# htcr/sam_road

Measured on AMD Instinct MI355X. Metric: tiles/sec (512x512 ViT-B, SAMRoad.infer_masks_and_img_features: encoder + mask decoder), higher is better.
Workload: dtype f16; 1 GPU; toponet_vitb_512_cityscale.yaml, batch=16 512x512 tiles per GPU, ViT-B encoder + map_decoder (BASELINE configs[1]); patch=512, input=f32 NHWC resident in HBM, weights=seeded random init, parallelism=tile-dp1

## Files before the change

include/samroad_hip.h:

```cpp
#ifndef SAMROAD_HIP_H
#define SAMROAD_HIP_H

#include <stddef.h>
#include <stdint.h>

#ifdef __cplusplus
extern "C" {
#endif

#define SRH_ABI_VERSION 11

typedef enum {
    SRH_OK = 0,
    SRH_ERR_BAD_ARG = -1,
    SRH_ERR_UNSUPPORTED = -2,
    SRH_ERR_HIP = -3,
    SRH_ERR_MISSING_WEIGHT = -4,
    SRH_ERR_NO_DEVICE = -5,
    SRH_ERR_NONFINITE = -6
} srh_status;

typedef enum { SRH_F32 = 0, SRH_F16 = 1, SRH_U8 = 2, SRH_I32 = 3, SRH_I64 = 4 } srh_dtype;

typedef struct srh_ctx srh_ctx;
// ... 68 lines not shown
                           int fill_b, void* stream);
int srh_scene_normalise_valid_hw(srh_ctx* ctx, const float* canvas_kp, const float* canvas_road, int H, int W,
                                 const int32_t* tile_xy, int n_tiles, int P, const uint8_t* valid, uint8_t* kp_u8,
                                 uint8_t* road_u8, void* stream);

int srh_scene_pass1_window_hw(srh_ctx* ctx, const srh_weights* w, const uint8_t* scene, int H, int W, const int32_t* tile_xy,
                              int n_tiles, int B, const float* profile, float* canvas_kp, float* canvas_road,
                              float* embeddings_all, void* stream);
int srh_scene_normalise_window_hw(srh_ctx* ctx, const float* canvas_kp, const float* canvas_road, int H, int W,
                                  const int32_t* tile_xy, int n_tiles, int P, const float* profile, const uint8_t* valid,
                                  uint8_t* kp_u8, uint8_t* road_u8, void* stream);
int srh_op_scene_fuse_window(srh_ctx* ctx, const float* scores, int n, int P, const int32_t* tile_xy, const float* profile,
                             float* canvas_kp, float* canvas_road, int H, int W, void* stream);

int srh_scene_pass1_tta_hw(srh_ctx* ctx, const srh_weights* w, const uint8_t* scene, int H, int W, const int32_t* tile_xy,
                           int n_tiles, int B, const uint8_t* orients, int k, const float* profile, float* canvas_kp,
                           float* canvas_road, float* embeddings_all, void* stream);
int srh_op_patch_im2col(srh_ctx* ctx, const uint8_t* scene_u8, int H, int W, const int32_t* tile_xy, int n, int P, int orient,
                        void* out_f16, void* stream);
int srh_op_scores_unorient(srh_ctx* ctx, const float* scores_in, int n, int P, int orient, float* scores_out, void* stream);


int srh_op_gemm(srh_ctx* ctx, const void* A_f16, const void* W_f16, const float* bias, const float* resid,
                int M, int N, int K, int act, float* out_f32, void* out_f16, void* stream);
#define SRH_GEMM_A_BLOCKED16 1
#define SRH_GEMM_OUT_BLOCKED16 2
int srh_op_gemm_ex(srh_ctx* ctx, const void* A_f16, const void* W_f16, const float* bias, const float* resid,
                   int M, int N, int K, int act, float* out_f32, void* out_f16, int flags, void* stream);
size_t srh_ctx_device_bytes(const srh_ctx* ctx);
int srh_op_conv3x3(srh_ctx* ctx, const void* A_f16, const void* W_f16, int B, int S, int C, int N,
                   float* out_f32, void* stream);
int srh_op_layernorm(srh_ctx* ctx, const float* x, const float* gamma, const float* beta, float eps, int M,
                     int D, int gelu, float* out_f32, void* out_f16, void* stream);
int srh_op_attention(srh_ctx* ctx, const void* qkv_f16, const void* relpos_h_f16, const void* relpos_w_f16,
                     const void* bias_qkv_f16, int B, int S, int heads, int win, void* out_f16, void* stream);
int srh_op_attention_hd(srh_ctx* ctx, const void* qkv_f16, const void* relpos_h_f16, const void* relpos_w_f16,
                        const void* bias_qkv_f16, int B, int S, int heads, int head_dim, int win,
                        void* out_f16, void* stream);

int srh_op_map_decoder(srh_ctx* ctx, const srh_weights* w, const void* emb_f16, int B, float* mask_logits, float* mask_scores, void* stream);
int srh_op_sample(srh_ctx* ctx, const float* emb_f32, int n_tiles, int h, int w, int C, const void* points, int points_dtype,
                  const int32_t* point_tile, int B, int N, float patch, float* out_f32, void* out_f16, void* stream);
int srh_op_pair_gather(srh_ctx* ctx, const void* pf_f16, const void* points, int points_dtype, const void* pairs, int pairs_dtype,
                       int B, int N, int Ns, int K, int zero_offset, int64_t index_base, void* out_f16, int ld, void* stream);


typedef struct {
    char name[32];
    int64_t launches;
    double ms;
    double flops;
    double bytes;
} srh_profile_row;
int srh_profile_enable(srh_ctx* ctx, int on);
int srh_profile_read(srh_ctx* ctx, srh_profile_row* rows, int max_rows, int* n_rows);
int srh_profile_overhead(srh_ctx* ctx, void* stream, double* ms_per_launch);

int srh_nms_points_host(const int32_t* xy, const uint8_t* force, int64_t n, int32_t radius, uint8_t* kept);

int srh_pass2_count(const int64_t* pts, int64_t n, const int32_t* boxes, int32_t n_tiles, int64_t* counts);
int srh_pass2_fill(const int64_t* pts, int64_t n, const int32_t* boxes, int32_t n_tiles, int32_t K, int64_t radius,
                   const int64_t* offsets, int64_t* ids, int32_t* knn, uint8_t* ambiguous, int64_t* local, int32_t n_threads);

int srh_kdtree_knn_host(const double* points, int64_t n, int32_t leafsize, const double* queries, int64_t nq, int32_t k,
                        double distance_upper_bound, int32_t* out_idx, int32_t* tree_indices);

// ... 32 lines not shown
```

sam_road_amd/_lib.py:

```python
import ctypes as C
import os

_HERE = os.path.dirname(os.path.abspath(__file__))
LIB_PATH = os.environ.get("SRH_LIB_PATH") or os.path.join(_HERE, "libsamroad_hip.so")

SRH_F32, SRH_F16, SRH_U8, SRH_I32, SRH_I64 = 0, 1, 2, 3, 4
ABI_VERSION = 11
SRH_GEMM_A_BLOCKED16, SRH_GEMM_OUT_BLOCKED16 = 1, 2


class SrhError(RuntimeError):
    pass


class ModelCfg(C.Structure):
    _fields_ = [("embed_dim", C.c_int32), ("depth", C.c_int32), ("num_heads", C.c_int32),
                ("patch_size", C.c_int32), ("n_global", C.c_int32), ("global_attn_indexes", C.c_int32 * 8),
                ("window_size", C.c_int32), ("toponet_version", C.c_int32), ("use_sam_decoder", C.c_int32)]


class NamedTensor(C.Structure):
    _fields_ = [("name", C.c_char_p), ("data", C.c_void_p), ("on_device", C.c_int32), ("ndim", C.c_int32),
                ("shape", C.c_int64 * 4)]

# ... 4 lines not shown


_P, _I, _F = C.c_void_p, C.c_int, C.c_float
SYMBOLS = {
    "srh_abi_version": (_I, []),
    "srh_build_id": (C.c_char_p, []),
    "srh_ctx_create": (_I, [_I, C.POINTER(_P)]),
    "srh_ctx_destroy": (None, [_P]),
    "srh_last_error": (C.c_char_p, [_P]),
    "srh_weights_pack": (_I, [_P, C.POINTER(ModelCfg), C.POINTER(NamedTensor), _I, C.POINTER(_P)]),
    "srh_weights_free": (None, [_P]),
    "srh_weights_export": (_I, [_P, _P, _P, C.c_size_t, C.POINTER(C.c_size_t)]),
    "srh_weights_import": (_I, [_P, C.POINTER(ModelCfg), _P, C.c_size_t, C.POINTER(_P)]),
    "srh_encode_decode": (_I, [_P, _P, _P, _I, _I, _P, _P, _P, _P]),
    "srh_toponet": (_I, [_P, _P, _P, _P, _I, _P, _I, _P, _I, _I, _I, _I, _P, _P, _P]),
    "srh_scene_pass1": (_I, [_P, _P, _P, _I, _P, _I, _I, _P, _P, _P, _P]),
    "srh_scene_normalise": (_I, [_P, _P, _P, _I, _P, _I, _I, _P, _P, _P]),
    "srh_scene_pass1_hw": (_I, [_P, _P, _P, _I, _I, _P, _I, _I, _P, _P, _P, _P]),
    "srh_scene_normalise_hw": (_I, [_P, _P, _P, _I, _I, _P, _I, _I, _P, _P, _P]),
    "srh_scene_tile_valid": (_I, [_P, _P, _I, _I, _P, _I, _I, _P, _P]),
    "srh_scene_fill_invalid": (_I, [_P, _P, _P, _I, _I, _I, _I, _I, _P]),
    "srh_scene_normalise_valid_hw": (_I, [_P, _P, _P, _I, _I, _P, _I, _I, _P, _P, _P, _P]),
    "srh_scene_pass1_window_hw": (_I, [_P, _P, _P, _I, _I, _P, _I, _I, _P, _P, _P, _P, _P]),
    "srh_scene_normalise_window_hw": (_I, [_P, _P, _P, _I, _I, _P, _I, _I, _P, _P, _P, _P, _P]),
    "srh_op_scene_fuse_window": (_I, [_P, _P, _I, _I, _P, _P, _P, _P, _I, _I, _P]),
    "srh_scene_pass1_tta_hw": (_I, [_P, _P, _P, _I, _I, _P, _I, _I, _P, _I, _P, _P, _P, _P, _P]),
    "srh_op_patch_im2col": (_I, [_P, _P, _I, _I, _P, _I, _I, _I, _P, _P]),
    "srh_op_scores_unorient": (_I, [_P, _P, _I, _I, _I, _P, _P]),
    "srh_op_gemm": (_I, [_P, _P, _P, _P, _P, _I, _I, _I, _I, _P, _P, _P]),
    "srh_op_gemm_ex": (_I, [_P, _P, _P, _P, _P, _I, _I, _I, _I, _P, _P, _I, _P]),
    "srh_ctx_device_bytes": (C.c_size_t, [_P]),
    "srh_op_conv3x3": (_I, [_P, _P, _P, _I, _I, _I, _I, _P, _P]),
    "srh_op_layernorm": (_I, [_P, _P, _P, _P, _F, _I, _I, _I, _P, _P, _P]),
    "srh_op_attention": (_I, [_P, _P, _P, _P, _P, _I, _I, _I, _I, _P, _P]),
    "srh_op_attention_hd": (_I, [_P, _P, _P, _P, _P, _I, _I, _I, _I, _I, _P, _P]),
    "srh_op_map_decoder": (_I, [_P, _P, _P, _I, _P, _P, _P]),
    "srh_op_sample": (_I, [_P, _P, _I, _I, _I, _I, _P, _I, _P, _I, _I, _F, _P, _P, _P]),
    "srh_op_pair_gather": (_I, [_P, _P, _P, _I, _P, _I, _I, _I, _I, _I, _I, C.c_int64, _P, _I, _P]),
    "srh_nms_points_host": (_I, [_P, _P, C.c_int64, C.c_int32, _P]),
    "srh_pass2_count": (_I, [_P, C.c_int64, _P, C.c_int32, _P]),
    "srh_pass2_fill": (_I, [_P, C.c_int64, _P, C.c_int32, C.c_int32, C.c_int64, _P, _P, _P, _P, _P, C.c_int32]),
    "srh_pass2_votes": (_I, [_P, C.c_int32, C.c_int64, C.c_int32, _P, _P, _P, C.c_int64, _P, _P, C.c_int64, _P]),
    "srh_pass2_vote_sums": (_I, [_P, _P, _P, _P, C.c_int32, C.c_int32, _P, C.c_int32, _P, _P, C.c_int64, _P, _P, _P, _P, C.c_int64, _P, C.c_int32]),
    "srh_votes_to_edges": (_I, [_P, _P, _P, _P, C.c_int64, C.c_int64, C.c_double, _P, _P]),
    "srh_pass2_pack": (_I, [_P, _P, _P, C.c_int32, C.c_int64, C.c_int32, _P, _P, _P]),
    "srh_pass2_pack_ragged": (_I, [_P, _P, _P, C.c_int32, C.c_int32, _P, _P, _P, _P]),
    "srh_toponet_ragged": (_I, [_P, _P, _P, _I, _P, _P, _P, _P, C.c_int64, _I, _P, _P, _P]),
    "srh_ctx_check": (_I, [_P, _P, _I]),
    "srh_kdtree_knn_host": (_I, [_P, C.c_int64, C.c_int32, _P, C.c_int64, C.c_int32, C.c_double, _P, _P]),
    "srh_mask_candidates": (_I, [_P, C.c_int32, C.c_int32, C.c_float, _P, _P, C.c_int64, _P, C.c_int32]),
    "srh_nms_merge_points": (_I, [_P, _P, C.c_int64, _P, _P, C.c_int64, _P, C.c_int32, _P, _P]),
    "srh_edge_vote_accumulate": (_I, [_P, _P, C.c_int64, _P, _P, _P, _P, _P]),
    "srh_edge_vote_accumulate_mt": (_I, [_P, _P, C.c_int64, _P, _P, _P, _P, _P, C.c_int32]),
    "srh_profile_enable": (_I, [_P, _I]),
    "srh_profile_read": (_I, [_P, C.POINTER(ProfileRow), _I, C.POINTER(_I)]),
    "srh_profile_overhead": (_I, [_P, _P, C.POINTER(C.c_double)]),
}

_lib = None


def build_id():
    return load().srh_build_id().decode()


def load():
# ... 57 lines not shown
```

sam_road_amd/build.py:

```python
import hashlib
import os
import subprocess
import sys
from concurrent.futures import ThreadPoolExecutor

HERE = os.path.dirname(os.path.abspath(__file__))
CSRC = os.path.join(HERE, "csrc")
LIB = os.path.join(HERE, "libsamroad_hip.so")
SOURCES = ["api.hip", "gemm.hip", "gemm_z192.hip", "norm.hip", "patch.hip", "attention.hip", "attention_hdx.hip", "decoder.hip", "scene_valid.hip", "scene_window.hip", "scene_tta.hip", "sam_decoder.hip", "topo.hip", "topo_fused.hip", "host_geom.hip"]
FLAGS = ["--offload-arch=gfx950", "-O3", "-std=c++17", "-fPIC", "-Wall", "-Wno-unused-function", "-Wno-unused-value", "-Wno-unused-result"]

FILE_FLAGS = {"attention.hip": ["-fno-honor-nans"], "attention_hdx.hip": ["-fno-honor-nans"]}


def _hipcc():
    for cand in (os.environ.get("HIPCC"), "/opt/rocm/bin/hipcc", "hipcc"):
        if cand and (os.path.isabs(cand) and os.path.exists(cand) or not os.path.isabs(cand)):
            return cand
    return "hipcc"


_MARK = b"SRH_BUILD_ID="


def source_id():
    h = hashlib.sha256()
    files = sorted(os.path.join(CSRC, f) for f in os.listdir(CSRC) if f.endswith((".hip", ".hpp", ".h", ".inc")))
    files.append(os.path.join(HERE, "..", "include", "samroad_hip.h"))
    for f in files:
        h.update(os.path.basename(f).encode() + b"\0")
        with open(f, "rb") as fh:
            h.update(fh.read())
        h.update(b"\0")
    h.update(" ".join(FLAGS + SOURCES + [f"{k}:{' '.join(v)}" for k, v in sorted(FILE_FLAGS.items())]).encode())
    return h.hexdigest()[:16]


def library_id(path=LIB):
    try:
        with open(path, "rb") as fh:
            data = fh.read()
    except OSError:
# ... 41 lines not shown
```

sam_road_amd/csrc/api.hip:

```cpp
#include <hip/hip_runtime.h>

#include <algorithm>
#include <cmath>
#include <cstdio>
#include <cstdlib>
#include <cstring>
#include <map>
#include <string>
#include <vector>

#include "../../include/samroad_hip.h"
#include "kernels.hpp"

using namespace srh;

struct DevBuf {
    void* p = nullptr;
    size_t cap = 0;
    int ensure(size_t bytes, double slack = 0.0) {
        if (bytes <= cap) return 0;
        if (p) hipFree(p);
        p = nullptr; cap = 0;
        const size_t want = bytes + (size_t)(bytes * slack);
        if (hipMalloc(&p, want) != hipSuccess) return SRH_ERR_HIP;
// ... 591 lines not shown

extern "C" int srh_weights_import(srh_ctx* c, const srh_model_cfg* cfg, const void* src, size_t bytes, srh_weights** out) {
    if (!c || !cfg || !src || !out) return fail(c, SRH_ERR_BAD_ARG, "srh_weights_import: null argument");
    return pack_impl(c, cfg, nullptr, 0, src, bytes, out);
}

extern "C" void srh_weights_free(srh_weights* w) {
    if (!w) return;
    if (w->arena) hipFree(w->arena);
    delete w;
}

static double attn_flops(int B, int S, int heads, int hd, int win) {
    if (win == S) return 4.0 * B * heads * (double)S * S * S * S * hd;
    const int nw = (S + win - 1) / win;
    double q = 0;
    for (int wy = 0; wy < nw; ++wy)
        for (int wx = 0; wx < nw; ++wx)
            q += (double)std::min(win, S - wy * win) * std::min(win, S - wx * win);
    return 4.0 * B * heads * q * win * win * hd;
}

static int ensure_encoder_ws(srh_ctx* c, const srh_weights* w, int B) {
    const size_t T = (size_t)B * w->S * w->S, D = w->D;
    int rc = 0;
    rc |= c->a0.ensure(T * 768 * 2);
    rc |= c->x.ensure(T * D * 4);
    rc |= c->xn16.ensure(T * D * 2);
    rc |= c->delta16.ensure(T * D * 2);
    rc |= c->delta16b.ensure(T * D * 2);
    rc |= c->qkv16.ensure(T * 3 * D * 2);
    rc |= c->attn16.ensure(T * D * 2);
    rc |= c->hid16.ensure(T * 4 * D * 2);
    rc |= c->n1.ensure(T * 256 * 4);
    rc |= c->n1_16.ensure(T * 256 * 2);
    rc |= c->n2.ensure(T * 256 * 4);
    rc |= c->emb16.ensure(T * 256 * 2);
    return rc ? fail(c, SRH_ERR_HIP, "workspace allocation failed") : 0;
}

#define TRY(expr) do { const int rc_ = (expr); if (rc_) return rc_; } while (0)
#define TRYK(c, cls, fl, by, s, call) do { const int rc_ = run(c, cls, fl, by, s, [&] { return (call); }); \
    if (rc_) return fail(c, rc_ == -2 ? SRH_ERR_UNSUPPORTED : SRH_ERR_HIP, std::string(cls) + ": kernel launch failed"); } while (0)

static int sam_decode(srh_ctx* c, const srh_weights* w, int B, const float* emb, float* logits, float* scores, hipStream_t s) {
    const int S = w->S, HW = S * S, R = B * 4, P = w->cfg.patch_size;
    const size_t T = (size_t)B * HW;
    const SdW& d = w->sd;
    int rc = 0;
    rc |= c->sd_keys.ensure(T * 256 * 4);  rc |= c->sd_keys16.ensure(T * 256 * 2);
    rc |= c->sd_k16.ensure(T * 128 * 2);   rc |= c->sd_v16.ensure(T * 128 * 2);  rc |= c->sd_a16.ensure(T * 128 * 2);
    rc |= c->sd_u0.ensure(T * 256 * 4);    rc |= c->sd_u0_16.ensure(T * 256 * 2); rc |= c->sd_u1_16.ensure(T * 4 * 128 * 2);
    rc |= c->sd_low.ensure((size_t)B * 2 * 16 * HW * 4);
    rc |= c->sd_tok.ensure((size_t)R * (256 * 8 + 2048 + 128 * 4) * 4 + (size_t)B * 3 * (256 * 2 + 32) * 4);
    if (rc) return fail(c, SRH_ERR_HIP, "SAM decoder workspace allocation failed");
    float* keys = c->sd_keys.as<float>();
    f16* keys16 = c->sd_keys16.as<f16>();
    float* tb = c->sd_tok.as<float>();
    float* q = tb;              float* t0 = tb + (size_t)R * 256; float* t1 = t0 + (size_t)R * 256; float* t2 = t1 + (size_t)R * 256;
    float* t3 = t2 + (size_t)R * 256; float* qn = t3 + (size_t)R * 256;
    float* hid = tb + (size_t)R * 256 * 8;
    float* s0 = hid + (size_t)R * 2048; float* s1 = s0 + (size_t)R * 128; float* s2 = s1 + (size_t)R * 128; float* s3 = s2 + (size_t)R * 128;
    float* hy0 = s3 + (size_t)R * 128; float* hy1 = hy0 + (size_t)B * 3 * 256; float* hyper = hy1 + (size_t)B * 3 * 256;

    auto lin = [&](const float* x, int ldx, const float* xadd, int add_rows, const float* W, const float* b, int rows, int N, int K,
                   int act, float* y, int ldy) -> int {
        SdLinearParams lp;
// ... 140 lines not shown
        TRY(block_ln(b.ln1_g, b.ln1_b, true, 2 * blk));
        GemmParams g;
        g.A = c->xn16.as<f16>(); g.lda = D; g.W = b.qkv_w; g.ldw = D; g.M = T; g.N = 3 * D; g.K = D;
        g.bias = b.qkv_b; g.out_f16 = c->qkv16.as<f16>(); g.ldc16 = 3 * D;
        TRY(gemm(c, "gemm_qkv", g, s));
        AttnParams ap;
        ap.table_h = b.rel_h; ap.table_w = b.rel_w;
        ap.qkv = c->qkv16.as<f16>(); ap.ld = 3 * D; ap.bias_qkv = b.qkv_b16;
        ap.out = c->attn16.as<f16>(); ap.ldo = D; ap.B = B; ap.S = S; ap.heads = heads; ap.hd = hd; ap.win = b.win;
        ap.scale = 1.0f / sqrtf((float)hd);
        TRYK(c, b.win == S ? "attn_global" : "attn_window", attn_flops(B, S, heads, hd, b.win), 0, s, launch_attention(ap, s));
        TRY(branch_gemm("gemm_proj", c->attn16.as<f16>(), D, b.proj_w, D, b.proj_b, false));
        TRY(block_ln(b.ln2_g, b.ln2_b, !defer_x, 2 * blk + 1));
        GemmParams g1;
        g1.A = c->xn16.as<f16>(); g1.lda = D; g1.W = b.fc1_w; g1.ldw = D; g1.M = T; g1.N = 4 * D; g1.K = D;
        g1.bias = b.fc1_b; g1.act = 1; g1.out_f16 = c->hid16.as<f16>(); g1.ldc16 = 4 * D;
        int hid_blocked = 0;
        {
            GemmParams t1 = g1, t2;
            t1.out_blocked16 = 1;
            t2.A = c->hid16.as<f16>(); t2.lda = 4 * D; t2.W = b.fc2_w; t2.ldw = 4 * D; t2.M = T; t2.N = D; t2.K = 4 * D; t2.bias = b.fc2_b;
            t2.out_f16 = c->delta16b.as<f16>(); t2.ldc16 = D; t2.a_blocked16 = 1;
            hid_blocked = z192_preferred(t1) && z192_preferred(t2);
        }
        g1.out_blocked16 = hid_blocked;
        TRY(gemm(c, "gemm_fc1", g1, s));
        TRY(branch_gemm("gemm_fc2", c->hid16.as<f16>(), 4 * D, b.fc2_w, 4 * D, b.fc2_b, true, hid_blocked));
    }
    {
        NormParams cast;
        cast.x = c->x.as<float>(); cast.M = T; cast.D = D; cast.out_f16 = c->xn16.as<f16>();
        int reads = 0;
        TRY(fold_pending(cast, reads));
        TRYK(c, "layernorm", 0, (double)T * D * (6 + 2 * reads), s, launch_layernorm(cast, s));
        GemmParams g;
        g.A = c->xn16.as<f16>(); g.lda = D; g.W = w->neck0_w; g.ldw = D; g.M = T; g.N = 256; g.K = D;
        g.out_f32 = c->n1.as<float>(); g.ldc = 256;
        TRY(gemm(c, "gemm_neck", g, s));
        NormParams ln;
        ln.x = c->n1.as<float>(); ln.M = T; ln.D = 256; ln.eps = 1e-6f; ln.gamma = w->neck1_g; ln.beta = w->neck1_b;
        ln.out_f16 = c->n1_16.as<f16>(); ln.nf = c->nf_dev; ln.nf_tag = NF_NECK;
        TRYK(c, "layernorm", 0, (double)T * 256 * 6, s, launch_layernorm(ln, s));
        GemmParams g3;
        g3.A = c->n1_16.as<f16>(); g3.lda = 256; g3.W = w->neck2_w; g3.ldw = 2304; g3.M = T; g3.N = 256; g3.K = 2304;
        g3.conv_S = S; g3.conv_C = 256; g3.out_f32 = c->n2.as<float>(); g3.ldc = 256;
        TRY(gemm(c, "gemm_neck", g3, s));
        ln.x = c->n2.as<float>(); ln.gamma = w->neck3_g; ln.beta = w->neck3_b;
        ln.out_f16 = c->emb16.as<f16>(); ln.out_f32 = emb; ln.nf_tag = NF_NECK + 1;
        TRYK(c, "layernorm", 0, (double)T * 256 * 10, s, launch_layernorm(ln, s));
    }
    if (!logits && !scores) return 0;
    if (w->cfg.use_sam_decoder) return sam_decode(c, w, B, emb, logits, scores, s);
    {
        DecodeFusedParams dp;
        dp.emb16 = c->emb16.as<f16>(); dp.frags = w->dec_frags; dp.prm = w->dec_prm; dp.B = B; dp.S = S;
        dp.logits = logits; dp.scores = scores; dp.nf = c->nf_dev; dp.nf_tag = NF_DECODER;
        const double fl = 2.0 * T * (256.0 * 512 + 4 * 128.0 * 256 + 16 * 64.0 * 128 + 64 * 32.0 * 8);
        TRYK(c, "map_decoder", fl, (double)T * 512 + (double)T * 256 * ((logits ? 8 : 0) + (scores ? 8 : 0)), s, launch_decode_fused(dp, s));
    }
    return 0;
}

extern "C" int srh_encode_decode(srh_ctx* c, const srh_weights* w, const void* rgb, int rgb_dtype, int B,
                                 float* mask_logits, float* mask_scores, float* embeddings, void* stream) {
    if (!c || !w || !rgb || !embeddings || B <= 0) return fail(c, SRH_ERR_BAD_ARG, "srh_encode_decode: bad argument");
    if (rgb_dtype != SRH_F32 && rgb_dtype != SRH_U8) return fail(c, SRH_ERR_BAD_ARG, "rgb dtype must be f32 or u8");
    TRY(nonfinite_check(c, "srh_encode_decode"));
    hipSetDevice(c->device);
    PatchParams pp;
    pp.src = rgb; pp.src_is_u8 = rgb_dtype == SRH_U8;
    return encode_batch(c, w, pp, B, mask_logits, mask_scores, embeddings, (hipStream_t)stream);
}

static int toponet_impl(srh_ctx* c, const srh_weights* w, const float* embeddings, const void* points,
                        int points_dtype, const void* pairs, int pairs_dtype, const uint8_t* valid, int B, int N,
// ... 284 lines not shown
    g.bias = bias; g.resid = resid; g.ldr = N; g.act = act;
    g.out_f32 = out_f32; g.ldc = N; g.out_f16 = (f16*)out_f16; g.ldc16 = N;
    g.a_blocked16 = (flags & SRH_GEMM_A_BLOCKED16) != 0; g.out_blocked16 = (flags & SRH_GEMM_OUT_BLOCKED16) != 0;
    return gemm(c, "gemm_op", g, (hipStream_t)stream);
}

extern "C" int srh_op_gemm(srh_ctx* c, const void* A, const void* W, const float* bias, const float* resid, int M,
                           int N, int K, int act, float* out_f32, void* out_f16, void* stream) {
    return srh_op_gemm_ex(c, A, W, bias, resid, M, N, K, act, out_f32, out_f16, 0, stream);
}

extern "C" int srh_op_conv3x3(srh_ctx* c, const void* A, const void* W, int B, int S, int C, int N, float* out_f32,
                              void* stream) {
    if (!c || !A || !W || !out_f32) return fail(c, SRH_ERR_BAD_ARG, "srh_op_conv3x3: null argument");
    hipSetDevice(c->device);
    GemmParams g;
    g.A = (const f16*)A; g.lda = C; g.W = (const f16*)W; g.ldw = 9 * C; g.M = B * S * S; g.N = N; g.K = 9 * C;
    g.conv_S = S; g.conv_C = C; g.out_f32 = out_f32; g.ldc = N;
    return gemm(c, "gemm_op", g, (hipStream_t)stream);
}

extern "C" int srh_op_layernorm(srh_ctx* c, const float* x, const float* gamma, const float* beta, float eps, int M,
                                int D, int gelu, float* out_f32, void* out_f16, void* stream) {
    if (!c || !x) return fail(c, SRH_ERR_BAD_ARG, "srh_op_layernorm: null argument");
    hipSetDevice(c->device);
    NormParams ln;
    ln.x = x; ln.M = M; ln.D = D; ln.gamma = gamma; ln.beta = beta; ln.eps = eps; ln.act = gelu;
    ln.out_f32 = out_f32; ln.out_f16 = (f16*)out_f16;
    hipStream_t s = (hipStream_t)stream;
    TRYK(c, "layernorm", 0, 0, s, launch_layernorm(ln, s));
    return 0;
}

extern "C" int srh_op_map_decoder(srh_ctx* c, const srh_weights* w, const void* emb_f16, int B, float* mask_logits, float* mask_scores,
                                  void* stream) {
    if (!c || !w || !emb_f16 || B <= 0) return fail(c, SRH_ERR_BAD_ARG, "srh_op_map_decoder: bad argument");
    if (w->cfg.use_sam_decoder || !w->dec_frags) return fail(c, SRH_ERR_UNSUPPORTED, "srh_op_map_decoder: the weights have no naive map_decoder");
    if (!mask_logits && !mask_scores) return 0;
    hipSetDevice(c->device);
    hipStream_t s = (hipStream_t)stream;
    DecodeFusedParams dp;
    dp.emb16 = (const f16*)emb_f16; dp.frags = w->dec_frags; dp.prm = w->dec_prm; dp.B = B; dp.S = w->S;
    dp.logits = mask_logits; dp.scores = mask_scores; dp.nf = c->nf_dev; dp.nf_tag = NF_DECODER;
    TRYK(c, "map_decoder", 0, 0, s, launch_decode_fused(dp, s));
    return 0;
}

extern "C" int srh_op_sample(srh_ctx* c, const float* emb_f32, int n_tiles, int h, int w, int C, const void* points, int points_dtype,
                             const int32_t* point_tile, int B, int N, float patch, float* out_f32, void* out_f16, void* stream) {
    if (!c || !emb_f32 || !points || (!out_f32 && !out_f16)) return fail(c, SRH_ERR_BAD_ARG, "srh_op_sample: null argument");
    if (points_dtype != SRH_I64 && points_dtype != SRH_F32) return fail(c, SRH_ERR_BAD_ARG, "srh_op_sample: points dtype must be i64 or f32");
    if (B < 0 || N < 0 || h <= 0 || w <= 0 || C <= 0 || C % 4 || n_tiles <= 0 || !(patch > 0.f))
        return fail(c, SRH_ERR_BAD_ARG, "srh_op_sample: bad sizes (C must be a multiple of 4)");
    if (!point_tile && B > n_tiles) return fail(c, SRH_ERR_BAD_ARG, "srh_op_sample: without point_tile, batch b samples tile b: B must be <= n_tiles");
    hipSetDevice(c->device);
    hipStream_t s = (hipStream_t)stream;
    SampleParams sp;
    sp.emb = emb_f32; sp.points = points; sp.points_i64 = points_dtype == SRH_I64; sp.B = B; sp.N = N;
    sp.h = h; sp.w = w; sp.C = C; sp.patch = patch; sp.out_f32 = out_f32; sp.out_f16 = (f16*)out_f16;
    sp.point_tile = point_tile; sp.n_tiles = n_tiles;
    TRYK(c, "bilinear_sample", 0, 0, s, launch_sample(sp, s));
    return 0;
}

extern "C" int srh_op_pair_gather(srh_ctx* c, const void* pf_f16, const void* points, int points_dtype, const void* pairs, int pairs_dtype,
                                  int B, int N, int Ns, int K, int zero_offset, int64_t index_base, void* out_f16, int ld, void* stream) {
// ... 106 lines not shown
```

sam_road_amd/csrc/kernels.hpp:

```cpp
#pragma once
#include <mutex>

#include "common.hpp"

namespace srh {

struct OncePerDevice {
    std::mutex mu;
    unsigned long long done = 0;
    template <class F> bool run(F&& fn) {
        int dev = 0;
        if (hipGetDevice(&dev) != hipSuccess) return false;
        const unsigned long long bit = 1ull << (dev & 63);
        std::lock_guard<std::mutex> lk(mu);
        if (done & bit) return true;
        if (!fn()) return false;
        done |= bit;
        return true;
    }
};

struct ZTileTables {
    static constexpr int SLOTS = 32, SLOT_TILES = 8192;
    struct Key { int M = 0, N = 0, lda = 0, ldw = 0, ldc = 0, blocked = 0; };
// ... 24 lines not shown
    int tile_gr = 0, prio_mode = 0;
    unsigned long long* dbg = nullptr;
    int variant = 0;
    int splitk = 0; float* split_ws = nullptr;
    int defer_reduce = 0;
    int a_blocked16 = 0, out_blocked16 = 0;
    ZTileTables* ztab = nullptr;
};
int launch_gemm(const GemmParams& p, hipStream_t s);
int gemm_splitk_factor(const GemmParams& p);
bool z192_supported(const GemmParams& p);
bool z192_preferred(const GemmParams& p);
int launch_gemm_z192(const GemmParams& p, hipStream_t s, int var = 0);
#ifdef SRH_TUNING
bool q192_supported(const GemmParams& p);
int launch_gemm_q192(const GemmParams& p, hipStream_t s, int ablation = 0);
int z192_var_count();
int z192_var_out_blocked(int var);
#endif

struct NormParams {
    const float* x = nullptr; int M = 0, D = 0;
    int x_period = 0;
    const float* gamma = nullptr; const float* beta = nullptr; float eps = 1e-6f;
    int act = 0;
    f16* out_f16 = nullptr; float* out_f32 = nullptr;
    const f16* delta16 = nullptr; float* x_out = nullptr;
    const f16* delta16b = nullptr;
    const float* slices = nullptr; int nslices = 0; size_t slice_stride = 0; const float* slice_bias = nullptr;
    unsigned* nf = nullptr; int nf_tag = 0;
};
int launch_layernorm(const NormParams& p, hipStream_t s);

struct PatchParams {
    const void* src = nullptr;
    int src_is_u8 = 0;
    int B = 0, P = 0;
    int scene_W = 0;
    const int* tile_xy = nullptr;
    f16* out = nullptr;
};
int launch_patch_im2col(const PatchParams& p, hipStream_t s);

struct AttnParams {
    const f16* qkv = nullptr; int ld = 0;
    const f16* table_h = nullptr;
    const f16* table_w = nullptr;
    const f16* bias_qkv = nullptr;
    f16* out = nullptr; int ldo = 0;
    int B = 0, S = 0, heads = 0, hd = 0, win = 0;
    float scale = 0.125f;
    int ablate = 0;
    unsigned hx_order[16] = {};
    void* scratch = nullptr;
};
constexpr size_t ATTN_SCRATCH_BYTES = 512 * 128;
int launch_attention(const AttnParams& p, hipStream_t s);
bool attention_g64_supported(const AttnParams& p);
int launch_attention_g64(const AttnParams& p, hipStream_t s);
bool attention_hdx_supported(const AttnParams& p);
int launch_attention_hdx(const AttnParams& p, hipStream_t s);

struct DecodeFusedParams {
    const f16* emb16 = nullptr;
    const char* frags = nullptr;
    const float* prm = nullptr;
// ... 74 lines not shown
```

Baseline: 3884 tiles/s.

## Fuse neck input fold, 1x1 projection GEMM and LayerNorm into one kernel

```diff
diff --git a/include/samroad_hip.h b/include/samroad_hip.h
--- a/include/samroad_hip.h
+++ b/include/samroad_hip.h
@@ -124,6 +124,9 @@
                    float* out_f32, void* stream);
 int srh_op_layernorm(srh_ctx* ctx, const float* x, const float* gamma, const float* beta, float eps, int M,
                      int D, int gelu, float* out_f32, void* out_f16, void* stream);
+int srh_op_neck_in_fused(srh_ctx* ctx, const float* x, const void* delta16_f16, const void* delta16b_f16, const float* slices, int nslices,
+                         const float* slice_bias, const void* W_f16, const float* gamma, const float* beta, int M, int D,
+                         void* out_f16, void* stream);
 int srh_op_attention(srh_ctx* ctx, const void* qkv_f16, const void* relpos_h_f16, const void* relpos_w_f16,
                      const void* bias_qkv_f16, int B, int S, int heads, int win, void* out_f16, void* stream);
 int srh_op_attention_hd(srh_ctx* ctx, const void* qkv_f16, const void* relpos_h_f16, const void* relpos_w_f16,
diff --git a/sam_road_amd/_lib.py b/sam_road_amd/_lib.py
--- a/sam_road_amd/_lib.py
+++ b/sam_road_amd/_lib.py
@@ -60,6 +60,7 @@
     "srh_ctx_device_bytes": (C.c_size_t, [_P]),
     "srh_op_conv3x3": (_I, [_P, _P, _P, _I, _I, _I, _I, _P, _P]),
     "srh_op_layernorm": (_I, [_P, _P, _P, _P, _F, _I, _I, _I, _P, _P, _P]),
+    "srh_op_neck_in_fused": (_I, [_P, _P, _P, _P, _P, _I, _P, _P, _P, _P, _I, _I, _P, _P]),
     "srh_op_attention": (_I, [_P, _P, _P, _P, _P, _I, _I, _I, _I, _P, _P]),
     "srh_op_attention_hd": (_I, [_P, _P, _P, _P, _P, _I, _I, _I, _I, _I, _P, _P]),
     "srh_op_map_decoder": (_I, [_P, _P, _P, _I, _P, _P, _P]),
diff --git a/sam_road_amd/build.py b/sam_road_amd/build.py
--- a/sam_road_amd/build.py
+++ b/sam_road_amd/build.py
@@ -7,7 +7,7 @@
 HERE = os.path.dirname(os.path.abspath(__file__))
 CSRC = os.path.join(HERE, "csrc")
 LIB = os.path.join(HERE, "libsamroad_hip.so")
-SOURCES = ["api.hip", "gemm.hip", "gemm_z192.hip", "norm.hip", "patch.hip", "attention.hip", "attention_hdx.hip", "decoder.hip", "scene_valid.hip", "scene_window.hip", "scene_tta.hip", "sam_decoder.hip", "topo.hip", "topo_fused.hip", "host_geom.hip"]
+SOURCES = ["api.hip", "gemm.hip", "gemm_z192.hip", "norm.hip", "neck_fused.hip", "patch.hip", "attention.hip", "attention_hdx.hip", "decoder.hip", "scene_valid.hip", "scene_window.hip", "scene_tta.hip", "sam_decoder.hip", "topo.hip", "topo_fused.hip", "host_geom.hip"]
 FLAGS = ["--offload-arch=gfx950", "-O3", "-std=c++17", "-fPIC", "-Wall", "-Wno-unused-function", "-Wno-unused-value", "-Wno-unused-result"]
 
 FILE_FLAGS = {"attention.hip": ["-fno-honor-nans"], "attention_hdx.hip": ["-fno-honor-nans"]}
diff --git a/sam_road_amd/csrc/api.hip b/sam_road_amd/csrc/api.hip
--- a/sam_road_amd/csrc/api.hip
+++ b/sam_road_amd/csrc/api.hip
@@ -647,7 +647,6 @@
     rc |= c->qkv16.ensure(T * 3 * D * 2);
     rc |= c->attn16.ensure(T * D * 2);
     rc |= c->hid16.ensure(T * 4 * D * 2);
-    rc |= c->n1.ensure(T * 256 * 4);
     rc |= c->n1_16.ensure(T * 256 * 2);
     rc |= c->n2.ensure(T * 256 * 4);
     rc |= c->emb16.ensure(T * 256 * 2);
@@ -854,15 +853,25 @@
         cast.x = c->x.as<float>(); cast.M = T; cast.D = D; cast.out_f16 = c->xn16.as<f16>();
         int reads = 0;
         TRY(fold_pending(cast, reads));
-        TRYK(c, "layernorm", 0, (double)T * D * (6 + 2 * reads), s, launch_layernorm(cast, s));
-        GemmParams g;
-        g.A = c->xn16.as<f16>(); g.lda = D; g.W = w->neck0_w; g.ldw = D; g.M = T; g.N = 256; g.K = D;
-        g.out_f32 = c->n1.as<float>(); g.ldc = 256;
-        TRY(gemm(c, "gemm_neck", g, s));
         NormParams ln;
-        ln.x = c->n1.as<float>(); ln.M = T; ln.D = 256; ln.eps = 1e-6f; ln.gamma = w->neck1_g; ln.beta = w->neck1_b;
+        ln.M = T; ln.D = 256; ln.eps = 1e-6f; ln.gamma = w->neck1_g; ln.beta = w->neck1_b;
         ln.out_f16 = c->n1_16.as<f16>(); ln.nf = c->nf_dev; ln.nf_tag = NF_NECK;
-        TRYK(c, "layernorm", 0, (double)T * 256 * 6, s, launch_layernorm(ln, s));
+        NeckInParams ni;
+        ni.x = cast.x; ni.M = T; ni.D = D; ni.delta16 = cast.delta16; ni.delta16b = cast.delta16b;
+        ni.slices = cast.slices; ni.nslices = cast.nslices; ni.slice_stride = cast.slice_stride; ni.slice_bias = cast.slice_bias;
+        ni.W = w->neck0_w; ni.gamma = ln.gamma; ni.beta = ln.beta; ni.eps = ln.eps; ni.out_f16 = ln.out_f16; ni.nf = ln.nf; ni.nf_tag = ln.nf_tag;
+        if (neck_in_fused_supported(ni)) {
+            TRYK(c, "gemm_neck", 2.0 * T * 256.0 * D, 0.0, s, launch_neck_in_fused(ni, s));
+        } else {
+            if (c->n1.ensure((size_t)T * 256 * 4)) return fail(c, SRH_ERR_HIP, "workspace allocation failed");
+            TRYK(c, "layernorm", 0, (double)T * D * (6 + 2 * reads), s, launch_layernorm(cast, s));
+            GemmParams g;
+            g.A = c->xn16.as<f16>(); g.lda = D; g.W = w->neck0_w; g.ldw = D; g.M = T; g.N = 256; g.K = D;
+            g.out_f32 = c->n1.as<float>(); g.ldc = 256;
+            TRY(gemm(c, "gemm_neck", g, s));
+            ln.x = c->n1.as<float>();
+            TRYK(c, "layernorm", 0, (double)T * 256 * 6, s, launch_layernorm(ln, s));
+        }
         GemmParams g3;
         g3.A = c->n1_16.as<f16>(); g3.lda = 256; g3.W = w->neck2_w; g3.ldw = 2304; g3.M = T; g3.N = 256; g3.K = 2304;
         g3.conv_S = S; g3.conv_C = 256; g3.out_f32 = c->n2.as<float>(); g3.ldc = 256;
@@ -1213,6 +1222,20 @@
     return 0;
 }
 
+extern "C" int srh_op_neck_in_fused(srh_ctx* c, const float* x, const void* delta16, const void* delta16b, const float* slices, int nslices,
+                                    const float* slice_bias, const void* W, const float* gamma, const float* beta, int M, int D,
+                                    void* out_f16, void* stream) {
+    if (!c || !x || !W || !gamma || !beta || !out_f16 || M <= 0) return fail(c, SRH_ERR_BAD_ARG, "srh_op_neck_in_fused: bad argument");
+    hipSetDevice(c->device);
+    NeckInParams ni;
+    ni.x = x; ni.M = M; ni.D = D; ni.delta16 = (const f16*)delta16; ni.delta16b = (const f16*)delta16b;
+    ni.slices = slices; ni.nslices = slices ? nslices : 0; ni.slice_stride = (size_t)M * D; ni.slice_bias = slice_bias;
+    ni.W = (const f16*)W; ni.gamma = gamma; ni.beta = beta; ni.eps = 1e-6f; ni.out_f16 = (f16*)out_f16; ni.nf = c->nf_dev; ni.nf_tag = NF_NECK;
+    hipStream_t s = (hipStream_t)stream;
+    TRYK(c, "gemm_op", 2.0 * M * 256.0 * D, 0.0, s, launch_neck_in_fused(ni, s));
+    return 0;
+}
+
 extern "C" int srh_op_map_decoder(srh_ctx* c, const srh_weights* w, const void* emb_f16, int B, float* mask_logits, float* mask_scores,
                                   void* stream) {
     if (!c || !w || !emb_f16 || B <= 0) return fail(c, SRH_ERR_BAD_ARG, "srh_op_map_decoder: bad argument");
diff --git a/sam_road_amd/csrc/kernels.hpp b/sam_road_amd/csrc/kernels.hpp
--- a/sam_road_amd/csrc/kernels.hpp
+++ b/sam_road_amd/csrc/kernels.hpp
@@ -80,6 +80,18 @@
 };
 int launch_layernorm(const NormParams& p, hipStream_t s);
 
+struct NeckInParams {
+    const float* x = nullptr; int M = 0, D = 0;
+    const f16* delta16 = nullptr; const f16* delta16b = nullptr;
+    const float* slices = nullptr; int nslices = 0; size_t slice_stride = 0; const float* slice_bias = nullptr;
+    const f16* W = nullptr;
+    const float* gamma = nullptr; const float* beta = nullptr; float eps = 1e-6f;
+    f16* out_f16 = nullptr;
+    unsigned* nf = nullptr; int nf_tag = 0;
+};
+bool neck_in_fused_supported(const NeckInParams& p);
+int launch_neck_in_fused(const NeckInParams& p, hipStream_t s);
+
 struct PatchParams {
     const void* src = nullptr;
     int src_is_u8 = 0;
diff --git a/sam_road_amd/csrc/neck_fused.hip b/sam_road_amd/csrc/neck_fused.hip
--- /dev/null
+++ b/sam_road_amd/csrc/neck_fused.hip
@@ -0,0 +1,227 @@
+#include "common.hpp"
+#include "kernels.hpp"
+
+namespace srh {
+
+namespace {
+constexpr int NK_BM = 64, NK_BN = 256, NK_BK = 64;
+constexpr int NK_WT = NK_BN * NK_BK * 2;
+constexpr int NK_XT = NK_BM * NK_BK * 4;
+constexpr int NK_DT = NK_BM * NK_BK * 2;
+constexpr int NK_RAW = NK_XT + 2 * NK_DT;
+constexpr int NK_OFF_RAW = 2 * NK_WT, NK_OFF_A16 = NK_OFF_RAW + 2 * NK_RAW;
+constexpr int NK_LDS = NK_OFF_A16 + 2 * NK_DT;
+static_assert(NK_BM * NK_BN * 4 <= NK_OFF_RAW, "the f32 staging image of the epilogue overlays the weight ring");
+
+__device__ __forceinline__ void neck_dma16(unsigned voff, const void* sbase, unsigned lds_wave_uniform) {
+    asm volatile("s_mov_b32 m0, %2\n\ts_nop 0\n\tglobal_load_lds_dwordx4 %0, %1" :: "v"(voff), "s"(sbase), "s"(lds_wave_uniform) : "memory");
+}
+template <int N> __device__ __forceinline__ void neck_wait_vmcnt() { asm volatile("s_waitcnt vmcnt(%0)" :: "n"(N) : "memory"); }
+}
+
+template <int NB, int NSL>
+__global__ __launch_bounds__(256) void neck_in_fused_kernel(NeckInParams p) {
+    static_assert(NB == 0 || NSL == 0, "either fp16 branches or split-K slices");
+    constexpr int PX = 4 + 2 * NB;
+    extern __shared__ __attribute__((aligned(16))) char smem[];
+    const unsigned lds0 = (unsigned)(unsigned long long)(__attribute__((address_space(3))) void*)smem;
+    const int tid = threadIdx.x, lane = tid & 63;
+    const int wave = __builtin_amdgcn_readfirstlane(tid >> 6);
+    const int m0 = blockIdx.x * NK_BM;
+    const int nk = p.D / NK_BK;
+
+    unsigned xoff[4], doff[2], woff[8];
+#pragma unroll
+    for (int i = 0; i < 4; ++i) {
+        const int r = (i * 4 + wave) * 4 + (lane >> 4);
+        xoff[i] = ((unsigned)min(m0 + r, p.M - 1) * (unsigned)p.D + (lane & 15) * 4) * 4u;
+    }
+#pragma unroll
+    for (int i = 0; i < 2; ++i) {
+        const int r = (i * 4 + wave) * 8 + (lane >> 3);
+        doff[i] = ((unsigned)min(m0 + r, p.M - 1) * (unsigned)p.D + (lane & 7) * 8) * 2u;
+    }
+#pragma unroll
+    for (int i = 0; i < 8; ++i) {
+        const int r = (i * 4 + wave) * 8 + (lane >> 3);
+        woff[i] = ((unsigned)r * (unsigned)p.D + ((lane & 7) ^ ((r >> 1) & 7)) * 8) * 2u;
+    }
+    auto dma_x = [&](int kt, int st) {
+        const unsigned d = lds0 + NK_OFF_RAW + st * NK_RAW + wave * 1024;
+        const char* xs = reinterpret_cast<const char*>(p.x) + (size_t)kt * (NK_BK * 4);
+#pragma unroll
+        for (int i = 0; i < 4; ++i) neck_dma16(xoff[i], xs, d + i * 4096);
+        if (NB >= 1) {
+            const char* ds = reinterpret_cast<const char*>(p.delta16) + (size_t)kt * (NK_BK * 2);
+#pragma unroll
+            for (int i = 0; i < 2; ++i) neck_dma16(doff[i], ds, d + NK_XT + i * 4096);
+        }
+        if (NB >= 2) {
+            const char* ds = reinterpret_cast<const char*>(p.delta16b) + (size_t)kt * (NK_BK * 2);
+#pragma unroll
+            for (int i = 0; i < 2; ++i) neck_dma16(doff[i], ds, d + NK_XT + NK_DT + i * 4096);
+        }
+    };
+    auto dma_w = [&](int kt, int st) {
+        const unsigned d = lds0 + st * NK_WT + wave * 1024;
+        const char* ws = reinterpret_cast<const char*>(p.W) + (size_t)kt * (NK_BK * 2);
+#pragma unroll
+        for (int i = 0; i < 8; ++i) neck_dma16(woff[i], ws, d + i * 4096);
+    };
+    f32x4 sl[NSL ? 4 : 1][NSL ? NSL : 1];
+    auto load_slices = [&](int kt) {
+#pragma unroll
+        for (int ps = 0; ps < (NSL ? 4 : 0); ++ps) {
+            const int q = ps * 256 + tid;
+            const float* sp = p.slices + (size_t)min(m0 + (q >> 4), p.M - 1) * p.D + kt * NK_BK + (q & 15) * 4;
+#pragma unroll
+            for (int z = 0; z < NSL; ++z) sl[ps][z] = *reinterpret_cast<const f32x4*>(sp + (size_t)z * p.slice_stride);
+        }
+    };
+
+    f32x16 acc[2][2];
+#pragma unroll
+    for (int i = 0; i < 2; ++i)
+#pragma unroll
+        for (int j = 0; j < 2; ++j)
+#pragma unroll
+            for (int r = 0; r < 16; ++r) acc[i][j][r] = 0.f;
+    const int frow = lane & 31, fhalf = lane >> 5;
+    const int fkey = (frow >> 1) & 7;
+    int foff[4];
+#pragma unroll
+    for (int ks = 0; ks < 4; ++ks) foff[ks] = frow * 128 + (((ks * 2 + fhalf) ^ fkey) << 4);
+
+    dma_x(0, 0);
+    dma_w(0, 0);
+    if (nk > 1) dma_x(1, 1);
+    load_slices(0);
+    for (int kt = 0; kt < nk; ++kt) {
+        const int st = kt & 1;
+        if (kt + 1 < nk) neck_wait_vmcnt<PX>(); else neck_wait_vmcnt<0>();
+        __syncthreads();
+        const char* raw = smem + NK_OFF_RAW + st * NK_RAW;
+        char* a16 = smem + NK_OFF_A16 + st * NK_DT;
+#pragma unroll
+        for (int ps = 0; ps < 4; ++ps) {
+            const int q = ps * 256 + tid, r = q >> 4, c = q & 15;
+            f32x4 v = *reinterpret_cast<const f32x4*>(raw + q * 16);
+            if constexpr (NSL > 0) {
+                f32x4 s = sl[ps][0];
+#pragma unroll
+                for (int z = 1; z < NSL; ++z) s += sl[ps][z];
+                s += *reinterpret_cast<const f32x4*>(p.slice_bias + kt * NK_BK + c * 4);
+                v = s + v;
+            }
+            if constexpr (NB >= 1) {
+                const f16x4 d = *reinterpret_cast<const f16x4*>(raw + NK_XT + q * 8);
+#pragma unroll
+                for (int e = 0; e < 4; ++e) v[e] += (float)d[e];
+            }
+            if constexpr (NB >= 2) {
+                const f16x4 d = *reinterpret_cast<const f16x4*>(raw + NK_XT + NK_DT + q * 8);
+#pragma unroll
+                for (int e = 0; e < 4; ++e) v[e] += (float)d[e];
+            }
+            const f16x4 h = {(f16)v[0], (f16)v[1], (f16)v[2], (f16)v[3]};
+            *reinterpret_cast<f16x4*>(a16 + r * 128 + ((((c >> 1) ^ ((r >> 1) & 7)) << 4) | ((c & 1) << 3))) = h;
+        }
+        __syncthreads();
+        if (kt + 1 < nk) dma_w(kt + 1, st ^ 1);
+        if (kt + 2 < nk) dma_x(kt + 2, st);
+        if (NSL > 0 && kt + 1 < nk) load_slices(kt + 1);
+        const char* sa = smem + NK_OFF_A16 + st * NK_DT;
+        const char* sw = smem + st * NK_WT + wave * (64 * 128);
+#pragma unroll
+        for (int ks = 0; ks < 4; ++ks) {
+            f16x8 fw[2], fx[2];
+#pragma unroll
+            for (int i = 0; i < 2; ++i) {
+                fw[i] = *reinterpret_cast<const f16x8*>(sw + foff[ks] + i * 4096);
+                fx[i] = *reinterpret_cast<const f16x8*>(sa + foff[ks] + i * 4096);
+            }
+#pragma unroll
+            for (int i = 0; i < 2; ++i)
+#pragma unroll
+                for (int j = 0; j < 2; ++j) acc[i][j] = mfma32(fw[i], fx[j], acc[i][j]);
+        }
+    }
+    __syncthreads();
+#pragma unroll
+    for (int j = 0; j < 2; ++j) {
+        const int r = j * 32 + frow;
+#pragma unroll
+        for (int i = 0; i < 2; ++i)
+#pragma unroll
+            for (int q = 0; q < 4; ++q) {
+                const int c = wave * 16 + i * 8 + 2 * q + fhalf;
+                const f32x4 t = {acc[i][j][4 * q], acc[i][j][4 * q + 1], acc[i][j][4 * q + 2], acc[i][j][4 * q + 3]};
+                *reinterpret_cast<f32x4*>(smem + r * 1024 + ((c ^ r) << 4)) = t;
+            }
+    }
+    __syncthreads();
+    float g[4], be[4];
+    {
+        const float4 tg = *reinterpret_cast<const float4*>(p.gamma + lane * 4), tb = *reinterpret_cast<const float4*>(p.beta + lane * 4);
+        g[0] = tg.x; g[1] = tg.y; g[2] = tg.z; g[3] = tg.w;
+        be[0] = tb.x; be[1] = tb.y; be[2] = tb.z; be[3] = tb.w;
+    }
+    const float inv_d = 1.0f / (float)NK_BN;
+    for (int rr = 0; rr < 16; rr += 4) {
+        float v[4][4];
+#pragma unroll
+        for (int r = 0; r < 4; ++r) {
+            const int row = wave * 16 + rr + r;
+            const f32x4 t = *reinterpret_cast<const f32x4*>(smem + row * 1024 + ((lane ^ row) << 4));
+            v[r][0] = t[0]; v[r][1] = t[1]; v[r][2] = t[2]; v[r][3] = t[3];
+        }
+#pragma unroll
+        for (int r = 0; r < 4; ++r) {
+            const int row = m0 + wave * 16 + rr + r;
+            float s = 0.f;
+#pragma unroll
+            for (int e = 0; e < 4; ++e) s += v[r][e];
+            const float mean = wave_sum(s) * inv_d;
+            float q = 0.f;
+#pragma unroll
+            for (int e = 0; e < 4; ++e) { v[r][e] -= mean; q += v[r][e] * v[r][e]; }
+            const float var = wave_sum(q) * inv_d;
+            if (row >= p.M) continue;
+            if (p.nf && !(var < INFINITY) && lane == 0) p.nf[p.nf_tag] = 1u;
+            const float rstd = rsqrtf(var + p.eps);
+#pragma unroll
+            for (int e = 0; e < 4; ++e) v[r][e] = v[r][e] * rstd * g[e] + be[e];
+            const f16x4 h = {(f16)v[r][0], (f16)v[r][1], (f16)v[r][2], (f16)v[r][3]};
+            *reinterpret_cast<f16x4*>(p.out_f16 + (size_t)row * NK_BN + lane * 4) = h;
+        }
+    }
+}
+
+bool neck_in_fused_supported(const NeckInParams& p) {
+    if (!p.x || !p.W || !p.gamma || !p.beta || !p.out_f16 || p.M <= 0) return false;
+    if (p.D % NK_BK != 0 || p.D < 2 * NK_BK) return false;
+    if ((unsigned long long)p.M * p.D * 4 >= (1ull << 32)) return false;
+    if (p.delta16b && !p.delta16) return false;
+    if (p.slices) return !p.delta16 && p.slice_bias && p.nslices >= 1 && p.nslices <= 4;
+    return true;
+}
+
+int launch_neck_in_fused(const NeckInParams& p, hipStream_t s) {
+    if (p.M <= 0) return 0;
+    if (!neck_in_fused_supported(p)) return -2;
+    typedef void (*kern_t)(NeckInParams);
+    static const kern_t kerns[7] = {neck_in_fused_kernel<0, 0>, neck_in_fused_kernel<1, 0>, neck_in_fused_kernel<2, 0>, neck_in_fused_kernel<0, 1>,
+                                    neck_in_fused_kernel<0, 2>, neck_in_fused_kernel<0, 3>, neck_in_fused_kernel<0, 4>};
+    static OncePerDevice opt_in;
+    if (!opt_in.run([] {
+            for (const kern_t k : kerns)
+                if (hipFuncSetAttribute(reinterpret_cast<const void*>(k), hipFuncAttributeMaxDynamicSharedMemorySize, NK_LDS) != hipSuccess) return false;
+            return true;
+        }))
+        return -3;
+    const kern_t k = p.slices ? kerns[2 + p.nslices] : kerns[(p.delta16 ? 1 : 0) + (p.delta16b ? 1 : 0)];
+    hipLaunchKernelGGL(k, dim3((p.M + NK_BM - 1) / NK_BM), dim3(256), NK_LDS, s, p);
+    return hipGetLastError() == hipSuccess ? 0 : -3;
+}
+
+}
```

After: 3892 tiles/s, median of 6. No clear change (+0.2%).
